# jperezrua/mfas

Measured on AMD Instinct MI355X. Metric: candidate-archs trained/sec (NTU inner loop), higher is better.
Workload: dtype f32

## Files before the change

mfas_amd/csrc/chain.hip.h:

```cpp
#pragma once
struct ChainArgs {
    const CandDev* cands;
    float* plane;
    int64_t plane_stride;
    const float* wt;
    float* stepbuf;
    mfas_table tab;
    const int32_t* order;
    int64_t pos_t;
    int32_t base_t, nvalid;
    int32_t gstep, epoch, E;
    int32_t yf_in_lds, vec_in_lds;
    AdamC ac;
    Geo g;
    DevStats* stats;
    int32_t* status;
    const float* pos_w;
    uint32_t* cellflag;
    uint32_t flag_target, _padf;
    int32_t yf_reduced, _padr;
    float* logits_out;
    const float* dlogits_in;
    float* xch;
    int32_t xpar, nsplit, ncand, _pads;
// ... 1514 lines not shown
template <int MB>
__device__ __forceinline__ void lean_res_load(const ChainArgs& a, const int bid, float* lds, LeanRes& rs) {
    const CandDev& cd = a.cands[bid];
    const LeanLds<MB> ll(lds, a.g);
    const int tid = threadIdx.x, lane = tid & 63, wave = tid >> 6;
    for (int e = tid; e < ll.nvec; e += CHAIN_THREADS)
        for (int pl = 0; pl < 3; ++pl) ll.vec_l[pl * ll.nvec + e] = a.plane[pl * a.plane_stride + cd.vec_off + e];
    if (wave < LEAN_OWN_TILES) {
        const int s = wave;
        const bool live = lean_own_live(cd, a.g, s);
        for (int pl = 0; pl < 3; ++pl) {
            f32x4 v = {0.f, 0.f, 0.f, 0.f};
            if (live) v = *reinterpret_cast<const f32x4*>(a.plane + pl * a.plane_stride + lean_own_off(cd, s) + lane * 4);
            *reinterpret_cast<f32x4*>(ll.own + (pl * LEAN_OWN_TILES + s) * 256 + lane * 4) = v;
        }
        f32x4 t = {0.f, 0.f, 0.f, 0.f};
        if (live) t = *reinterpret_cast<const f32x4*>(a.wt + lean_own_toff(cd, s) + lane * 4);
        *reinterpret_cast<f32x4*>(ll.own + (3 * LEAN_OWN_TILES + s) * 256 + lane * 4) = t;
    }
    if (tid == CHAIN_THREADS - 64) { rs.loss = 0.0; rs.corr = 0; rs.bad = 0; }
    if (tid < 16) reinterpret_cast<uint32_t*>(ll.scr + LEAN_BNF)[tid] = 0u;
    __syncthreads();
}

template <int MB>
__device__ __forceinline__ void lean_res_update(const ChainArgs& a, const ChainStep& cs, const int bid, float* lds) {
    const CandDev& cd = a.cands[bid];
    const Geo& g = a.g;
    const LeanLds<MB> ll(lds, g);
    constexpr int Bp = MB * 16, SX = 20;
    const int tid = threadIdx.x, lane = tid & 63, wave = tid >> 6;
    const int l15 = lane & 15, lg = lane >> 4;
    const int L = cd.L;
    int s = -1;
    const float* x = nullptr;
    const float* dy = nullptr;
    int sx = SX, sd = SX, dcol = 0;
    if (wave >= 1 && wave < L) { s = wave - 1; x = ll.xo_l + (wave - 1) * Bp * SX; dy = ll.dy_l + wave * Bp * SX; }
    else if (wave >= 4 && wave - 4 < g.ncb) { s = 3 + (wave - 4); x = ll.xo_l + (L - 1) * Bp * SX; dy = ll.lg_l; sd = ll.SC; dcol = (wave - 4) * 16; }
    if (s >= 0) {
        float* oW = ll.own + s * 256 + lane * 4;
        float* oM = oW + LEAN_OWN_TILES * 256;
        float* oV = oM + LEAN_OWN_TILES * 256;
        f32x4 w4 = *reinterpret_cast<const f32x4*>(oW), m4 = *reinterpret_cast<const f32x4*>(oM), v4 = *reinterpret_cast<const f32x4*>(oV);
        f32x4 acc = {0.f, 0.f, 0.f, 0.f};
        DW_BATCH_LOOP(MB, (g.B + 3) >> 2, acc = MFMA16(x[(4 * j + lg) * sx + l15], dy[(4 * j + lg) * sd + dcol + l15], acc))
        const float gsc = 1.0f;
        adam4(w4, m4, v4, acc * gsc, cs.ss, cs.bc2s, a.ac.w1, a.ac.b2, a.ac.w2, a.ac.eps, a.ac.wd);
        *reinterpret_cast<f32x4*>(oW) = w4;
        *reinterpret_cast<f32x4*>(oM) = m4;
        *reinterpret_cast<f32x4*>(oV) = v4;
        float* oT = ll.own + (3 * LEAN_OWN_TILES + s) * 256;
        const int base = (((l15 >> 2) * 16 + 4 * lg) << 2) + (l15 & 3);
#pragma unroll
        for (int q = 0; q < 4; ++q) oT[base + 4 * q] = w4[q];
    }
    lds_barrier();
}

template <int MB>
__device__ __forceinline__ void lean_res_store(const ChainArgs& a, const int bid, const int epoch, float* lds, const LeanRes& rs) {
    const CandDev& cd = a.cands[bid];
    const LeanLds<MB> ll(lds, a.g);
    const int tid = threadIdx.x, lane = tid & 63, wave = tid >> 6;
    __syncthreads();
    for (int e = tid; e < ll.nvec; e += CHAIN_THREADS)
        for (int pl = 0; pl < 3; ++pl) a.plane[pl * a.plane_stride + cd.vec_off + e] = ll.vec_l[pl * ll.nvec + e];
    if (wave < LEAN_OWN_TILES && lean_own_live(cd, a.g, wave)) {
        const int s = wave;
        for (int pl = 0; pl < 3; ++pl)
            *reinterpret_cast<f32x4*>(a.plane + pl * a.plane_stride + lean_own_off(cd, s) + lane * 4) =
                *reinterpret_cast<const f32x4*>(ll.own + (pl * LEAN_OWN_TILES + s) * 256 + lane * 4);
        *reinterpret_cast<f32x4*>(const_cast<float*>(a.wt) + lean_own_toff(cd, s) + lane * 4) =
            *reinterpret_cast<const f32x4*>(ll.own + (3 * LEAN_OWN_TILES + s) * 256 + lane * 4);
    }
    if (tid == CHAIN_THREADS - 64) {
        DevStats& st = a.stats[(int64_t)cd.gidx * a.E + epoch];
        st.train_loss += rs.loss;
        st.train_corr += rs.corr;
        if (rs.bad) atomicMax(&a.status[cd.gidx], 1);
    }
}

#define XCH_SLOTS 7
#define XCH_SENT 0xFFFFFFFFu
#define XCH_SPIN_LIMIT (1u << 21)
#define XCH_CAND_FLOATS (2 * XCH_SLOTS * 8 * 256)

__device__ __forceinline__ f32x4 xch_wait(const float* base, const int64_t idx, int32_t* status, const int gidx) {
    uint32_t spins = 0;
    for (;;) {
        const f32x4 v = ldc4<true>(base, idx);
        const u32x4 u = __builtin_bit_cast(u32x4, v);
        if (u[0] != XCH_SENT && u[1] != XCH_SENT && u[2] != XCH_SENT && u[3] != XCH_SENT) return v;
        if (++spins > XCH_SPIN_LIMIT) { atomicMax(&status[gidx], 2); return v; }
        asm volatile("" ::: "memory");
        __builtin_amdgcn_s_sleep(1);
    }
}

template <int NS> __host__ __device__ constexpr size_t chain_split_lds_floats(int Rp, int Cp) {
    return (size_t)2 * 16 * (Rp + 4) + (size_t)16 * (Cp + 4) + (size_t)MFAS_MAX_CELLS * (8 / NS) * 16 + 48 + 16 +
           (size_t)MFAS_MAX_CELLS * (8 / NS) * 256 + (size_t)(MFAS_MAX_CELLS * 5 * (8 / NS) * 16 + Cp) + (size_t)(8 / NS) * 8 * 256 +
           (size_t)2 * MFAS_MAX_CELLS * (8 / NS) * 256 + (size_t)(8 / NS) * 256;
}

template <int NS>
__device__ __forceinline__ void chain_split(const ChainArgs& a, const ChainStep& cs, const int bid, const int part, float* lds) {
#ifdef MFAS_CHAIN_TIMING
    const unsigned long long ct0 = __builtin_readcyclecounter();
#define CS_STAMP(slot) do { if (threadIdx.x == 0 && bid == 0 && part == 0 && cs.gstep == 3) a.status[64 + (slot)] = (int32_t)(__builtin_readcyclecounter() - ct0); } while (0)
    if (threadIdx.x == 0 && bid == 0 && part == 0 && (cs.gstep == 3 || cs.gstep == 4)) a.status[64 + 23 + 2 * (cs.gstep - 3)] = (int32_t)wall_clock64();
#else
#define CS_STAMP(slot) do { } while (0)
#endif
    constexpr int NRO = 8 / NS;
    constexpr int Bp = 16, MB = 1;
    const CandDev& cd = a.cands[bid];
    const Geo& g = a.g;
    const int tid = threadIdx.x, lane = tid & 63, wave = tid >> 6;
    const int l15 = lane & 15, lg = lane >> 4;
    const int Rp = g.Rp, nrb = 8, Cp = g.Cp, ncb = g.ncb, R = g.R, C = g.C, L = cd.L;
    const int SX = Rp + 4, SC = Cp + 4;
    constexpr int LPR = 16;
    float* xo_l = lds;
    float* dy_l = xo_l;
    float* lg_l = xo_l + 2 * Bp * SX;
    float* rstd_l = lg_l + Bp * SC;
    float* red_l = rstd_l + MFAS_MAX_CELLS * (8 / NS) * 16;
    int* lab_l = reinterpret_cast<int*>(red_l + 48);
    float* yf_l = reinterpret_cast<float*>(lab_l + 16);
    constexpr int NCOL = NRO * 16;
    float* vl = yf_l + MFAS_MAX_CELLS * NRO * 256;
    const int nvec = MFAS_MAX_CELLS * 5 * NCOL;
    const int vplane = nvec + Cp;
    float* tb = vl + vplane;
    float* sv_l = tb + NRO * 8 * 256;
    float* odd_l = sv_l + 2 * MFAS_MAX_CELLS * NRO * 256;

    float* W = a.plane;
    float* Mv = a.plane + a.plane_stride;
    float* Vv = Mv + a.plane_stride;
    float* sb = a.stepbuf + cd.step_off;
    const int64_t cvec_off = cd.vec_off;
    int nlbits = 0;
#pragma unroll
    for (int i = 0; i < MFAS_MAX_CELLS; ++i) nlbits |= (cd.conf[i][2] & 3) << (2 * i);
    const int cgidx = cd.gidx;
    asm volatile("" :: "s"(nlbits), "s"(cgidx));
    CS_STAMP(34);
    const int64_t oP1 = cd.seg_off[1][2], oP2 = cd.seg_off[2][2], oP3 = cd.seg_off[3][2];
    const int64_t oT1 = cd.outT_off[1], oT2 = cd.outT_off[2], oT3 = cd.outT_off[3], oHT = cd.headT_off;
    auto offP = [&](const int i) { return i == 1 ? oP1 : (i == 2 ? oP2 : oP3); };
    auto offT = [&](const int i) { return i == 1 ? oT1 : (i == 2 ? oT2 : oT3); };
    const int nvalid = cs.nvalid;
    const float nf = (float)nvalid;
    const AdamC ac = adam_consts(a.ac, cs.ss, cs.bc2s);
    const uint32_t h0 = lowbias32(cd.drop_seed + 0x9E3779B9U * (uint32_t)(cs.gstep + 1));
    const int64_t sbo = cd.step_off;
    const int rb0 = part * NRO;
    const bool main_w = wave < NRO;
    const int rb = rb0 + (main_w ? wave : 0);
    const int64_t xq = (int64_t)cgidx * XCH_CAND_FLOATS;
    const int64_t xcur_par = xq + (int64_t)a.xpar * (XCH_SLOTS * 8 * 256);
    const int64_t xoth_par = xq + (int64_t)(a.xpar ^ 1) * (XCH_SLOTS * 8 * 256);

    f32x4 hw[4];
    const int hcb = wave & 3, hpar = wave >> 2;
    const bool head_w = hcb < ncb;
#pragma unroll
    for (int u = 0; u < 4; ++u) {
        hw[u] = (f32x4){0.f, 0.f, 0.f, 0.f};
        if (head_w) hw[u] = *reinterpret_cast<const f32x4*>(W + cd.head_off + ((int64_t)hcb * nrb + 2 * u + hpar) * 256 + lane * 4);
    }
    f32x4 stg[NRO];
    auto stage_issue = [&](const float* base, const int64_t off0, const int nk) {
#pragma unroll
        for (int u = 0; u < NRO; ++u) {
            const int e = wave + 8 * u;
            const int j = e / nk, k = e - j * nk;
            if (e < NRO * nk) stg[u] = *reinterpret_cast<const f32x4*>(base + off0 + ((int64_t)(rb0 + j) * nk + k) * 256 + lane * 4);
        }
    };
    auto stage_store = [&](float* dst, const int nk) {
#pragma unroll
        for (int u = 0; u < NRO; ++u) {
            const int e = wave + 8 * u;
            const int j = e / nk, k = e - j * nk;
            if (e < NRO * nk) *as_lds(reinterpret_cast<f32x4*>(dst + (j * 8 + k) * 256 + lane * 4)) = stg[u];
        }
// ... 86 lines not shown
            const int u = 2 * u2 + odd;
            if (u < nk) {
                const f32x4 w4 = *as_lds(reinterpret_cast<const f32x4*>(tiles + u * 256 + lane * 4));
                const f32x4 x4 = *reinterpret_cast<const f32x4*>(X + l15 * sx + u * 16 + 4 * lg);
#pragma unroll
                for (int q = 0; q < 4; ++q) acc = MFMA16(x4[q], w4[q], acc);
            }
        }
    };
    const bool help_w = wave >= NRO && wave < 2 * NRO;
    static_assert(2 * (8 / NS) <= 4, "main + helper waves below the head waves");
    const int vcol = (main_w ? wave : 0) * 16 + l15;

    for (int i = 0; i < L; ++i) {
        CS_STAMP(1 + i);
        if (i == L - 1 && lab_b >= 0 && lab_b < Bp && lab_b < nvalid) lab_r = g.loss_mode == 0 ? a.tab.label[lab_row] : (int)lab_row;
        const bool st_fw = i + 1 < L && i >= 1;
        const bool st_hd = i + 1 == L;
        if (st_fw) stage_issue(W, offP(i + 1), nrb);
        else if (st_hd) stage_issue(a.wt, oHT, ncb);
        const float* xprev = xo_l + ((i + 1) & 1) * Bp * SX;
        float* xcur = xo_l + (i & 1) * Bp * SX;
        if (main_w) {
            const int nl = (nlbits >> (2 * i)) & 3;
            const int64_t vb = cvec_off + (int64_t)i * g.vec_cell_stride;
            const float* vc = vl + i * 5 * NCOL;
            const int r = rb * 16 + l15;
            const bool colok = r < R;
            const float bias = vc[VEC_B * NCOL + vcol];
            float gam = 1.f, bet = 0.f;
            if (g.bn) { gam = vc[VEC_G * NCOL + vcol]; bet = vc[VEC_BE * NCOL + vcol]; }
            f32x4 acc = *as_lds(reinterpret_cast<const f32x4*>(yf_l + ((i * NRO + wave) << 8) + lane * 4));
            if (i > 0) {
                mma_half(acc, xprev, SX, tb + wave * 8 * 256, nrb, 0);
                lds_barrier();
                acc += *as_lds(reinterpret_cast<const f32x4*>(odd_l + wave * 256 + lane * 4));
            }
            if (i == 1) CS_STAMP(13);
            float av[4];
            float s = 0.f;
#pragma unroll
            for (int q = 0; q < 4; ++q) {
                const int b = 4 * lg + q;
                const float v = act_fwd(acc[q] + bias, nl);
                av[q] = v;
                if (b < nvalid) s += v;
            }
            float zv[4];
            if (g.bn) {
                const float mu = colsum(s) / nf;
                float s2 = 0.f;
#pragma unroll
                for (int q = 0; q < 4; ++q) {
                    const int b = 4 * lg + q;
                    const float dlt = av[q] - mu;
                    if (b < nvalid) s2 += dlt * dlt;
                }
                const float var = colsum(s2) / nf;
                const float rstd = 1.0f / sqrtf(var + g.bn_eps);
                f32x4 xh4;
#pragma unroll
                for (int q = 0; q < 4; ++q) {
                    const float xh = (av[q] - mu) * rstd;
                    xh4[q] = xh;
                    zv[q] = xh * gam + bet;
                }
                if (lg == 0) {
                    rstd_l[i * NCOL + vcol] = rstd;
                    if (colok) {
                        float rm = vc[VEC_RM * NCOL + vcol], rv = vc[VEC_RV * NCOL + vcol];
                        const float unb = var * (nf / (nf - 1.0f));
                        rm += g.bn_mom * (mu - rm);
                        rv += g.bn_mom * (unb - rv);
                        W[vb + VEC_RM * Rp + r] = rm;
                        W[vb + VEC_RV * Rp + r] = rv;
                    }
                }
                *as_lds(reinterpret_cast<f32x4*>(sv_l + ((MFAS_MAX_CELLS + i) * NRO + wave) * 256 + lane * 4)) = xh4;
            } else {
#pragma unroll
                for (int q = 0; q < 4; ++q) zv[q] = av[q];
            }
            *as_lds(reinterpret_cast<f32x4*>(sv_l + (i * NRO + wave) * 256 + lane * 4)) = (f32x4){av[0], av[1], av[2], av[3]};
            float* xo_g = sb + g.sb_xo + (int64_t)i * Bp * Rp;
            f32x4 o4;
#pragma unroll
            for (int q = 0; q < 4; ++q) {
                const int b = 4 * lg + q;
                float o = zv[q];
                if (g.use_drop) o = ((keepm >> (4 * i + q)) & 1u) ? o * g.drop_scale : 0.0f;
                if (!(colok && b < nvalid)) o = 0.0f;
                o4[q] = o;
            }
            stc4<true>(a.xch, xcur_par + ((int64_t)i * 8 + rb) * 256 + lane * 4, o4);
            if (i == 1) CS_STAMP(14);
            if (i + 1 < L) keep_bits(i + 1);
#pragma unroll
            for (int q = 0; q < 4; ++q) {
                const int b = 4 * lg + q;
                xcur[b * SX + r] = o4[q];
                stc1<true>(xo_g + b * Rp + r, o4[q]);
            }
        }
        if (!main_w && i > 0) {
            if (help_w) {
                f32x4 acc2 = {0.f, 0.f, 0.f, 0.f};
                mma_half(acc2, xprev, SX, tb + (wave - NRO) * 8 * 256, nrb, 1);
                *as_lds(reinterpret_cast<f32x4*>(odd_l + (wave - NRO) * 256 + lane * 4)) = acc2;
            }
            lds_barrier();
        }
        if (st_fw) stage_store(tb, nrb);
        else if (st_hd) stage_store(tb, ncb);
        if (i == 1) CS_STAMP(15);
        fetch_others(i, xcur);
        if (i == 1) CS_STAMP(16);
        lds_barrier();
    }

    CS_STAMP(5);
    {
        const float* xl = xo_l + ((L - 1) & 1) * Bp * SX;
        float* hodd = xo_l + (L & 1) * Bp * SX;
        f32x4 acc = {0.f, 0.f, 0.f, 0.f};
        if (head_w) {
#pragma unroll
            for (int u = 0; u < 4; ++u) {
                const f32x4 x4 = *reinterpret_cast<const f32x4*>(xl + l15 * SX + (2 * u + hpar) * 16 + 4 * lg);
#pragma unroll
                for (int q = 0; q < 4; ++q) acc = MFMA16(x4[q], hw[u][q], acc);
            }
            if (hpar) *as_lds(reinterpret_cast<f32x4*>(hodd + hcb * 256 + lane * 4)) = acc;
        }
        lds_barrier();
        if (head_w && !hpar) {
            acc += *as_lds(reinterpret_cast<const f32x4*>(hodd + hcb * 256 + lane * 4));
            const int c = hcb * 16 + l15;
            const float bias = vl[nvec + c];
#pragma unroll
            for (int q = 0; q < 4; ++q) lg_l[(4 * lg + q) * SC + c] = acc[q] + bias;
        }
    }
    if (lab_b >= 0 && lab_b < Bp) lab_l[lab_b] = lab_r;
    lds_barrier();
    CS_STAMP(6);
    if (g.loss_mode == 1) {
        if (tid < 4 * Bp) bce_rows(lg_l, SC, red_l, Bp, lab_l, a.tab.multilabel, a.pos_w, C, Cp, nvalid, tid);
    } else if (Cp <= 64 && !g.multitask) {
        if (tid < 8 * Bp) softmax_rows_lean<MB>(a, lg_l, SC, red_l, lab_l, nvalid, nf, tid);
    } else if (tid < LPR * Bp) {
        softmax_rows<MB>(a, cs, lg_l, SC, red_l, lab_l, nvalid, nf, tid, cand_order(a.order, g, cgidx));
    }
    CS_STAMP(21);
    lds_barrier();
    if (part == 0) {
        if (tid == CHAIN_THREADS - 64 && a.stats) {
            float ls = 0.f, ncor = 0.f;
            for (int b = 0; b < Bp; ++b) { ls += red_l[b]; ncor += red_l[Bp + b]; }
            DevStats& st = a.stats[(int64_t)cgidx * a.E + cs.epoch];
            st.train_loss += (double)ls;
            st.train_corr += (long long)ncor;
            if (!(fabsf(ls) <= 3.0e38f)) atomicMax(&a.status[cgidx], 1);
        }
        float* dlg = sb + g.sb_dlog;
        for (int e = tid; e < Bp * Cp; e += CHAIN_THREADS) {
            const int b = e / Cp, c = e - b * Cp;
            stc1<true>(dlg + e, lg_l[b * SC + c]);
        }
        const int hc = tid - (CHAIN_THREADS - 256);
        if (hc >= 0 && hc < C) {
            float gsum = 0.f;
            for (int b = 0; b < Bp; ++b) gsum += lg_l[b * SC + hc];
            const int64_t o = cvec_off + g.vec_head + hc;
            float w = vl[nvec + hc], m = Mv[o], v = Vv[o];
            adam1(w, m, v, gsum, ac);
            W[o] = w; Mv[o] = m; Vv[o] = v;
        }
    }
    CS_STAMP(7);

    for (int i = L - 1; i >= 0; --i) {
        CS_STAMP(8 + (L - 1 - i));
        const int j = L - 1 - i;
        const bool st_bw = i >= 1;
        if (st_bw) stage_issue(a.wt, offT(i), nrb);
        const bool from_head = (i == L - 1);
        const float* src = from_head ? lg_l : dy_l + ((i + 1) & 1) * Bp * SX;
        const int sstride = from_head ? SC : SX;
        const int nkk = from_head ? ncb : nrb;
        float* dcur = dy_l + (i & 1) * Bp * SX;
        if (main_w) {
            const int nl = (nlbits >> (2 * i)) & 3;
            const int64_t vb = cvec_off + (int64_t)i * g.vec_cell_stride;
            const float* vc = vl + i * 5 * NCOL;
            const int r = rb * 16 + l15;
            const bool colok = r < R;
            float gr = 0.f;
            if (g.bn) gr = vc[VEC_G * NCOL + vcol] * rstd_l[i * NCOL + vcol];
            const int64_t ob = vb + VEC_B * Rp + r, og = vb + VEC_G * Rp + r, obe = vb + VEC_BE * Rp + r;
            float pw[3] = {0.f, 0.f, 0.f}, pm[3] = {0.f, 0.f, 0.f}, pv[3] = {0.f, 0.f, 0.f};
            if (lg == 0 && colok) {
                pw[0] = vc[VEC_B * NCOL + vcol]; pm[0] = Mv[ob]; pv[0] = Vv[ob];
                if (g.bn) {
                    pw[1] = vc[VEC_G * NCOL + vcol]; pm[1] = Mv[og]; pv[1] = Vv[og];
                    pw[2] = vc[VEC_BE * NCOL + vcol]; pm[2] = Mv[obe]; pv[2] = Vv[obe];
                }
            }
            const f32x4 a4 = *as_lds(reinterpret_cast<const f32x4*>(sv_l + (i * NRO + wave) * 256 + lane * 4));
            f32x4 xh4 = {0.f, 0.f, 0.f, 0.f};
            if (g.bn) xh4 = *as_lds(reinterpret_cast<const f32x4*>(sv_l + ((MFAS_MAX_CELLS + i) * NRO + wave) * 256 + lane * 4));
            f32x4 acc = {0.f, 0.f, 0.f, 0.f};
            mma_half(acc, src, sstride, tb + wave * 8 * 256, nkk, 0);
            lds_barrier();
            acc += *as_lds(reinterpret_cast<const f32x4*>(odd_l + wave * 256 + lane * 4));
            if (i == 2) CS_STAMP(17);
            float dz[4];
            float sdz = 0.f, sdzx = 0.f;
#pragma unroll
            for (int q = 0; q < 4; ++q) {
                const int b = 4 * lg + q;
                float d = acc[q];
                if (g.use_drop) d = ((keepm >> (4 * i + q)) & 1u) ? d * g.drop_scale : 0.0f;
                if (!(b < nvalid)) d = 0.f;
                dz[q] = d;
                sdz += d;
                if (g.bn) sdzx += d * xh4[q];
            }
            float dgam = 0.f, dbet = 0.f;
            if (g.bn) {
                dbet = colsum(sdz);
                dgam = colsum(sdzx);
                const float k1 = dbet / nf, k2 = dgam / nf;
#pragma unroll
                for (int q = 0; q < 4; ++q) {
                    const int b = 4 * lg + q;
                    const float da = gr * (dz[q] - k1 - xh4[q] * k2);
                    dz[q] = b < nvalid ? da : 0.f;
                }
            }
            float sdy = 0.f;
            float* dy_g = sb + g.sb_dy + (int64_t)i * Bp * Rp;
            f32x4 d4;
#pragma unroll
            for (int q = 0; q < 4; ++q) {
                float dy = act_bwd(a4[q], dz[q], nl);
                if (!colok) dy = 0.f;
                sdy += dy;
                d4[q] = dy;
            }
            if (i >= 1) stc4<true>(a.xch, xcur_par + ((int64_t)(4 + j) * 8 + rb) * 256 + lane * 4, d4);
            if (i == 2) CS_STAMP(18);
#pragma unroll
            for (int q = 0; q < 4; ++q) {
                const int b = 4 * lg + q;
                dcur[b * SX + r] = d4[q];
                stc1<true>(dy_g + b * Rp + r, d4[q]);
            }
            const float db = colsum(sdy);
            if (lg == 0 && colok) {
                adam1(pw[0], pm[0], pv[0], db, ac);
                W[ob] = pw[0]; Mv[ob] = pm[0]; Vv[ob] = pv[0];
                if (g.bn) {
                    adam1(pw[1], pm[1], pv[1], dgam, ac);
                    W[og] = pw[1]; Mv[og] = pm[1]; Vv[og] = pv[1];
                    adam1(pw[2], pm[2], pv[2], dbet, ac);
                    W[obe] = pw[2]; Mv[obe] = pm[2]; Vv[obe] = pv[2];
                }
            }
        }
        if (!main_w) {
            if (help_w) {
                f32x4 acc2 = {0.f, 0.f, 0.f, 0.f};
                mma_half(acc2, src, sstride, tb + (wave - NRO) * 8 * 256, nkk, 1);
                *as_lds(reinterpret_cast<f32x4*>(odd_l + (wave - NRO) * 256 + lane * 4)) = acc2;
            }
            lds_barrier();
        }
        if (st_bw) stage_store(tb, nrb);
        if (i == 2) CS_STAMP(19);
        if (i >= 1) fetch_others(4 + j, dcur);
        if (i == 2) CS_STAMP(20);
        asm volatile("s_waitcnt vmcnt(0)" ::: "memory");
        lds_barrier();
        if (a.cellflag && tid == 0)
            __hip_atomic_fetch_add(a.cellflag + (size_t)cgidx * CELLFLAG_STRIDE + i, 1u, __ATOMIC_RELAXED, __HIP_MEMORY_SCOPE_AGENT);
    }
    CS_STAMP(12);
#ifdef MFAS_CHAIN_TIMING
    if (threadIdx.x == 0 && bid == 0 && part == 0 && (cs.gstep == 3 || cs.gstep == 4)) a.status[64 + 24 + 2 * (cs.gstep - 3)] = (int32_t)wall_clock64();
#endif
#undef CS_STAMP
}
```

mfas_amd/csrc/common.hip.h:

```cpp
#pragma once

typedef float f32x4 __attribute__((ext_vector_type(4)));
typedef int32_t i32x4 __attribute__((ext_vector_type(4)));
typedef uint32_t u32x4 __attribute__((ext_vector_type(4)));
typedef uint32_t u32x2 __attribute__((ext_vector_type(2)));
#define MFAS_LDS __attribute__((address_space(3)))
#define MFAS_GLB __attribute__((address_space(1)))
template <typename T> __device__ __forceinline__ MFAS_LDS T* as_lds(T* p) { return (MFAS_LDS T*)p; }
template <typename T> __device__ __forceinline__ MFAS_GLB T* as_glb(T* p) { return (MFAS_GLB T*)p; }
#define MFMA16(a, b, c) __builtin_amdgcn_mfma_f32_16x16x4f32((a), (b), (c), 0, 0, 0)

#define KIND_S 0
#define KIND_V 1
#define KIND_OUT 2
#define KIND_HEAD 3

static thread_local std::string g_err;
static int fail(int code, const std::string& msg) {
    g_err = msg;
    return code;
}
#define HIPCHK(x)                                                                                  \
    do {                                                                                           \
        hipError_t e_ = (x);                                                                       \
// ... 247 lines not shown
    if (dtype == MFAS_DT_F32) {
        const int vpr = ncols >> 2;
        for (int e = tid; e < nrows * vpr; e += nthreads) {
            const int b = e / vpr, c = (e - b * vpr) << 2;
            f32x4 val = {0.f, 0.f, 0.f, 0.f};
            if (b < nvalid) {
                const int64_t row = ord ? (int64_t)ord[pos + b] : (int64_t)(base + b);
                val = *reinterpret_cast<const f32x4*>(reinterpret_cast<const float*>(tab) + row * width + col0 + c);
            }
            *as_lds(reinterpret_cast<f32x4*>(dst + b * stride + c)) = val;
        }
    } else {
        const int vpr = ncols >> 3;
        for (int e = tid; e < nrows * vpr; e += nthreads) {
            const int b = e / vpr, c = (e - b * vpr) << 3;
            f32x4 lo = {0.f, 0.f, 0.f, 0.f}, hi = {0.f, 0.f, 0.f, 0.f};
            if (b < nvalid) {
                const int64_t row = ord ? (int64_t)ord[pos + b] : (int64_t)(base + b);
                const uint4 raw = *reinterpret_cast<const uint4*>(reinterpret_cast<const uint16_t*>(tab) +
                                                                  row * width + col0 + c);
                const uint32_t w[4] = {raw.x, raw.y, raw.z, raw.w};
                float f[8];
#pragma unroll
                for (int j = 0; j < 4; ++j) {
                    if (dtype == MFAS_DT_BF16) {
                        f[2 * j] = __uint_as_float(w[j] << 16);
                        f[2 * j + 1] = __uint_as_float(w[j] & 0xFFFF0000U);
                    } else {
                        f[2 * j] = __half2float(__ushort_as_half((unsigned short)(w[j] & 0xFFFFU)));
                        f[2 * j + 1] = __half2float(__ushort_as_half((unsigned short)(w[j] >> 16)));
                    }
                }
                lo = (f32x4){f[0], f[1], f[2], f[3]};
                hi = (f32x4){f[4], f[5], f[6], f[7]};
            }
            *as_lds(reinterpret_cast<f32x4*>(dst + b * stride + c)) = lo;
            *as_lds(reinterpret_cast<f32x4*>(dst + b * stride + c + 4)) = hi;
        }
    }
}

typedef unsigned u32x4 __attribute__((ext_vector_type(4)));
#define MFAS_AUX_SC1 16
__device__ __forceinline__ __amdgpu_buffer_rsrc_t mk_rsrc(const float* base) {
    return __builtin_amdgcn_make_buffer_rsrc(const_cast<float*>(base), 0, -1, 0x00020000);
}
template <bool COH>
__device__ __forceinline__ f32x4 ldc4(const float* base, int64_t idx) {
    if constexpr (COH) {
        const u32x4 r = __builtin_amdgcn_raw_buffer_load_b128(mk_rsrc(base), (int)(uint32_t)(idx << 2), 0, MFAS_AUX_SC1);
        return __builtin_bit_cast(f32x4, r);
    } else {
        return *reinterpret_cast<const f32x4*>(base + idx);
    }
}
template <bool COH>
__device__ __forceinline__ void stc4(float* base, int64_t idx, f32x4 v) {
    if constexpr (COH)
        __builtin_amdgcn_raw_buffer_store_b128(__builtin_bit_cast(u32x4, v), mk_rsrc(base), (int)(uint32_t)(idx << 2), 0, MFAS_AUX_SC1);
    else
        *reinterpret_cast<f32x4*>(base + idx) = v;
}
template <bool COH>
__device__ __forceinline__ void stc1(float* p, float v) {
    if constexpr (COH) __hip_atomic_store(p, v, __ATOMIC_RELAXED, __HIP_MEMORY_SCOPE_AGENT);
    else *p = v;
}
template <bool COH>
__device__ __forceinline__ float ldc1(const float* p) {
    if constexpr (COH) return __hip_atomic_load(p, __ATOMIC_RELAXED, __HIP_MEMORY_SCOPE_AGENT);
    else return *p;
}

template <bool COH>
__device__ __forceinline__ void stage_f32(float* dst, int stride, const float* base, int64_t idx0, int src_stride, int ncols,
                                          int nrows, int tid, int nthreads) {
    const int vpr = ncols >> 2;
    for (int e = tid; e < nrows * vpr; e += nthreads) {
        const int b = e / vpr, c = (e - b * vpr) << 2;
        *reinterpret_cast<f32x4*>(dst + b * stride + c) = ldc4<COH>(base, idx0 + (int64_t)b * src_stride + c);
    }
}

template <int MB, int WPE> struct SweepU { static constexpr int v = (MB == 2 && WPE == 4) ? 1 : 2; };
```

mfas_amd/csrc/mfas_hip.hip:

```cpp
#include <hip/hip_runtime.h>
#include <hip/hip_fp16.h>
#pragma clang fp contract(off)
#include <stdint.h>
#include <stdio.h>
#include <string.h>
#include <math.h>
#include <algorithm>
#include <string>
#include <vector>
#include <thread>
#include <chrono>
#include <dlfcn.h>

#include "mfas_hip.h"

#include "common.hip.h"
#include "sweep.hip.h"
#include "chain.hip.h"

struct StepArgs {
    SweepArgs sa;
    ChainArgs ca;
    int32_t nchain, _pad;
    GatherArgs ga;
};

template <int MB, bool NT, int WPE, bool LEAN, int NS = 1>
__global__ void __launch_bounds__(STEP_THREADS, WPE) k_step(const StepArgs a) {
    extern __shared__ __attribute__((aligned(16))) float lds[];
    const int bid = (int)blockIdx.x;
    if (bid < a.nchain) {
        if constexpr (NS > 1) {
            const int Kp = a.nchain / NS, part = bid / Kp, c = bid - part * Kp;
            if (c < a.ca.ncand) chain_split<NS>(a.ca, chain_step_of(a.ca), c, part, lds);
        } else
        if constexpr (LEAN) { chain_lean<MB, 0, (WPE >= 4 ? 8 : 16)>(a.ca, chain_step_of(a.ca), bid, lds, lean_pre<MB>(a.ca, bid)); chain_lean_tail<MB, 0>(a.ca, chain_step_of(a.ca), bid, lds); }
        else chain_body<MB, false>(a.ca, chain_step_of(a.ca), bid, lds);
    }
    else if (bid < a.nchain + a.ga.nblocks) gather_body(a.ga, a.ga.cands[bid - a.nchain], a.sa.g, a.sa.tab, a.sa.order, (int)threadIdx.x);
    else if (bid < a.nchain + a.ga.nblocks + a.sa.ntap) sweep_tap_body<MB, NT, SweepU<MB, WPE>::v>(a.sa, bid - a.nchain - a.ga.nblocks, lds);
    else sweep_body<MB, NT, SweepU<MB, WPE>::v>(a.sa, sweep_step_of(a.sa), bid - a.nchain - a.ga.nblocks - a.sa.ntap, lds);
}

template <int MB, bool NT, int NS = 1>
__global__ void __launch_bounds__(STEP_THREADS, 4) k_step_same(const StepArgs a) {
    extern __shared__ __attribute__((aligned(16))) float lds[];
    const int bid = (int)blockIdx.x;
    if (bid < a.nchain) {
        if constexpr (NS > 1) {
            const int Kp = a.nchain / NS, part = bid / Kp, c = bid - part * Kp;
            if (c < a.ca.ncand) chain_split<NS>(a.ca, chain_step_of(a.ca), c, part, lds);
        } else chain_body<MB, false, true>(a.ca, chain_step_of(a.ca), bid, lds);
    } else sweep_body<MB, NT, SweepU<MB, 4>::v, true>(a.sa, sweep_step_of(a.sa), bid - a.nchain, lds);
}

template <int MB, bool LEAN>
__global__ void __launch_bounds__(STEP_THREADS, 2) k_chain(const ChainArgs a) {
    extern __shared__ __attribute__((aligned(16))) float lds[];
    if constexpr (LEAN) { chain_lean<MB>(a, chain_step_of(a), (int)blockIdx.x, lds, lean_pre<MB>(a, (int)blockIdx.x)); chain_lean_tail<MB, 0>(a, chain_step_of(a), (int)blockIdx.x, lds); }
    else chain_body<MB, true>(a, chain_step_of(a), (int)blockIdx.x, lds);
}

#include "wide.hip.h"
#include "persist.hip.h"
#include "eval.hip.h"
#include "pack.hip.h"

#include "plan.hip.h"

struct mfas_population {
    mfas_hyper hp;
    Tuning tune;
    int K = 0, device = 0, n_cus = 0;
    int chunk_cols_req = 0;
    hipStream_t stream = nullptr;
    LayoutPlan plan;
    float* plane = nullptr;
    float* wt = nullptr;
    float* stepbuf = nullptr;
    float* best = nullptr;
    CandDev* d_cands = nullptr;
    SegDesc* d_descs = nullptr;
    struct GroupDev { SegDesc* d_descs = nullptr; TapDesc* d_taps = nullptr; };
    std::vector<GroupDev> groups;
    DevStats* d_stats = nullptr;
    int32_t* d_status = nullptr;
    uint32_t* d_seeds = nullptr;
    long long* d_corr = nullptr;
    float* d_posw = nullptr;
    int stats_cap = 0;
    bool profiling = false;
    int prof_every = 16;
    std::vector<hipEvent_t> ev;
    int64_t prof_launches = 0;
    double prof_ms = 0.0, bytes_per_launch = 0.0, prof_bytes = 0.0;
    double best_threshold = 0.0;
    struct Progress {
        std::vector<int64_t> done, nb;
        std::vector<double> best_metric;
        std::vector<int32_t> keeps_best;
        void reset(int K, double threshold) { done.assign(K, 0); nb.assign(K, 0); best_metric.assign(K, threshold); keeps_best.assign(K, 0); }
    } prog;
    float* d_move = nullptr;
    int64_t move_cap = 0;
    uint32_t* d_red_cnt = nullptr;
    char* d_gather = nullptr;
    size_t gather_cap = 0;
    uint32_t* d_cellflag = nullptr;
    float* d_xch = nullptr;
    SegDesc* d_pdescs = nullptr;
    int fell_back = 0;
    uint32_t* d_sync = nullptr;
    int32_t* d_need = nullptr;
    int32_t* d_role = nullptr;
    float* d_scal = nullptr;
    size_t scal_cap = 0;
    unsigned long long* d_trace = nullptr;
};

namespace {
struct Roctx {
    int (*push)(const char*) = nullptr;
    int (*pop)() = nullptr;
    Roctx() {
        if (getenv("MFAS_NO_ROCTX")) return;
        void* h = dlopen("librocprofiler-sdk-roctx.so", RTLD_LAZY | RTLD_LOCAL);
        if (!h) h = dlopen("librocprofiler-sdk-roctx.so.1", RTLD_LAZY | RTLD_LOCAL);
        if (!h) h = dlopen("libroctx64.so", RTLD_LAZY | RTLD_LOCAL);
        if (!h) return;
        push = reinterpret_cast<int (*)(const char*)>(dlsym(h, "roctxRangePushA"));
        pop = reinterpret_cast<int (*)()>(dlsym(h, "roctxRangePop"));
        if (!push || !pop) { push = nullptr; pop = nullptr; }
    }
};
Roctx& roctx() { static Roctx r; return r; }
struct RangeGuard {
// ... 460 lines not shown
```

mfas_amd/csrc/sweep.hip.h:

```cpp
#pragma once
template <int MB, bool NT, int SWEEP_U, bool COH = false>
__device__ __forceinline__ void tile_run(float* Wp, float* Mp, float* Vp, const int rb, const int nkb, const int kb0,
                                         const int kbs, const float* xt, const int ST, const float* xn, const int SN,
                                         const float (&dyf)[MB * 4], const float gsc, const AdamC& ac, const bool upd,
                                         const bool fwd, f32x4 (&yacc)[MB], float* T, const int tstride_rb,
                                         const int lane, const int nj) {
    const int l15 = lane & 15, lg = lane >> 4;
    const float a_ss = ac.ss, a_bc2s = ac.bc2s, a_w1 = ac.w1, a_b2 = ac.b2, a_w2 = ac.w2, a_eps = ac.eps, a_wd = ac.wd;
    for (int kbb = kb0; kbb < nkb; kbb += SWEEP_U * kbs) {
        f32x4 w4[SWEEP_U], m4[SWEEP_U], v4[SWEEP_U];
#pragma unroll
        for (int u = 0; u < SWEEP_U; ++u) {
            const int kb = kbb + u * kbs;
            if (kb < nkb) {
                const int64_t off = ((int64_t)rb * nkb + kb) * 256 + lane * 4;
                w4[u] = NT ? __builtin_nontemporal_load(reinterpret_cast<const f32x4*>(Wp + off))
                           : *reinterpret_cast<const f32x4*>(Wp + off);
                if (upd) {
                    m4[u] = NT ? __builtin_nontemporal_load(reinterpret_cast<const f32x4*>(Mp + off))
                               : *reinterpret_cast<const f32x4*>(Mp + off);
                    v4[u] = NT ? __builtin_nontemporal_load(reinterpret_cast<const f32x4*>(Vp + off))
                               : *reinterpret_cast<const f32x4*>(Vp + off);
                }
            }
// ... 69 lines not shown
__device__ __forceinline__ int64_t gather_tap_off(const Geo& g, const int kind, const int tap, const int eb) {
    int64_t o = 0;
#pragma unroll
    for (int u = 0; u < MFAS_MAX_TAPS; ++u) {
        if (kind == KIND_V || u < tap) o += g.sw[u];
        if (kind == KIND_V && u < tap) o += g.vw[u];
    }
    return o * g.Bp * eb;
}

struct GatherArgs {
    const CandDev* cands;
    char* buf;
    int64_t cand_stride, par_stride;
    int64_t pos[2];
    int32_t base[2], nvalid[2], par[2];
    int32_t nsets, nblocks;
};

__device__ __forceinline__ void gather_body(const GatherArgs& ga, const CandDev& cd, const Geo& g, const mfas_table& tab,
                                            const int32_t* order, const int tid) {
    const int eb = tab.dtype == MFAS_DT_F32 ? 4 : 2;
    const int32_t* ordp = cand_order(order, g, cd.gidx);
    uint32_t used = 0;
    for (int i = 0; i < cd.L; ++i) used |= (1u << cd.conf[i][0]) | (1u << (MFAS_MAX_TAPS + cd.conf[i][1]));
#pragma unroll
    for (int s = 0; s < 2; ++s) {
        if (s >= ga.nsets) break;
        char* dst0 = ga.buf + (int64_t)cd.gidx * ga.cand_stride + (int64_t)ga.par[s] * ga.par_stride;
        for (int kt = 0; kt < 2 * MFAS_MAX_TAPS; ++kt) {
            if (!((used >> kt) & 1u)) continue;
            const int kind = kt < MFAS_MAX_TAPS ? KIND_S : KIND_V, tap = kt & (MFAS_MAX_TAPS - 1);
            const int w = kind == KIND_S ? g.sw[tap] : g.vw[tap];
            const char* src0 = reinterpret_cast<const char*>(kind == KIND_S ? tab.s[tap] : tab.v[tap]);
            char* dst = dst0 + gather_tap_off(g, kind, tap, eb);
            const int vpr = (w * eb) >> 4, nvec = ga.nvalid[s] * vpr;
            for (int e0 = tid; e0 < nvec; e0 += 4 * STEP_THREADS) {
                u32x4 v[4];
#pragma unroll
                for (int u = 0; u < 4; ++u) {
                    const int e = e0 + u * STEP_THREADS;
                    if (e < nvec) {
                        const int b = e / vpr, c = e - b * vpr;
                        const int64_t row = ordp ? (int64_t)ordp[ga.pos[s] + b] : (int64_t)(ga.base[s] + b);
                        v[u] = *reinterpret_cast<const u32x4*>(src0 + (row * w) * eb + ((int64_t)c << 4));
                    }
                }
#pragma unroll
                for (int u = 0; u < 4; ++u) {
                    const int e = e0 + u * STEP_THREADS;
                    if (e < nvec) {
                        const int b = e / vpr, c = e - b * vpr;
                        *reinterpret_cast<u32x4*>(dst + ((int64_t)b * w) * eb + ((int64_t)c << 4)) = v[u];
                    }
                }
            }
        }
    }
}

struct SweepStep {
    int64_t pos_t, pos_n;
    int32_t base_t, base_n, nvalid_t, nvalid_n;
    int32_t upd, fwd;
    float ss, bc2s;
};
__device__ __forceinline__ SweepStep sweep_step_of(const SweepArgs& a) {
    SweepStep s;
    s.pos_t = a.pos_t; s.pos_n = a.pos_n; s.base_t = a.base_t; s.base_n = a.base_n;
    s.nvalid_t = a.nvalid_t; s.nvalid_n = a.nvalid_n; s.upd = a.do_update; s.fwd = a.do_forward;
    s.ss = a.ac.ss; s.bc2s = a.ac.bc2s;
    return s;
}


#ifdef MFAS_CHAIN_TIMING
#define SW_UNIT_STAMP(k) do { if (COH && a.cellflag && a.flag_target == 16u && threadIdx.x == 0 && d.cell == 0 && d.kind == KIND_S && d.k0 == 0 && d.cand == 0) a.flag_status[64 + 29 + (k)] = (int32_t)wall_clock64(); } while (0)
#define SW_END_STAMP() do { if (COH && a.cellflag && a.flag_target == 16u && threadIdx.x == 0) { atomicMax(reinterpret_cast<uint32_t*>(&a.flag_status[64 + 27]), (uint32_t)wall_clock64()); \
        atomicMax(reinterpret_cast<uint32_t*>(&a.flag_status[128 + d.cell * 4 + d.kind]), (uint32_t)wall_clock64()); } } while (0)
#else
#define SW_END_STAMP() do { } while (0)
#define SW_UNIT_STAMP(k) do { } while (0)
#endif
template <int MB, bool NT, int U, bool COH = false>
__device__ __forceinline__ void sweep_body(const SweepArgs& a, const SweepStep& st, const int bid, float* lds) {
    const SegDesc d = a.desc[bid];
    const CandDev& cd = a.cands[d.cand];
    const int tid = threadIdx.x, lane = tid & 63, wave = tid >> 6;
    const int l15 = lane & 15, lg = lane >> 4;
    constexpr int Bp = MB * 16;
    const int cc = d.cc, rows_p = d.rows_p, nrb = rows_p >> 4, nkb = cc >> 4;
    const int ST = cc + 16;
    const int SN = cc + 4;
    const int SD = rows_p + 16;
    float* xt = lds;
    float* xn = xt + Bp * ST;
    float* dyl = xn + Bp * SN;
    float* wred = dyl + Bp * SD;
    const bool feat = d.kind <= KIND_V;
    const bool upd = st.upd != 0;
    const bool fwd = (st.fwd != 0) && feat;
    if (!upd && !fwd) return;
    const int64_t sbo = cd.step_off;
    const bool red = a.red_cnt != nullptr;

    if (!COH && a.gather && feat) {
        const char* gb = a.gather + (int64_t)cd.gidx * a.g_cand_stride + gather_tap_off(a.g, d.kind, d.tap, a.tab.dtype == MFAS_DT_F32 ? 4 : 2);
        if (upd) stage_table(xt, ST, gb + (int64_t)a.g_par_t * a.g_par_stride, a.tab.dtype, d.width, d.k0, cc, nullptr, 0, 0, st.nvalid_t, Bp, tid, STEP_THREADS);
        if (fwd) stage_table(xn, SN, gb + (int64_t)a.g_par_n * a.g_par_stride, a.tab.dtype, d.width, d.k0, cc, nullptr, 0, 0, st.nvalid_n, Bp, tid, STEP_THREADS);
    } else {
    if (upd && feat) {
        const void* tp = d.kind == KIND_S ? a.tab.s[d.tap] : a.tab.v[d.tap];
        stage_table(xt, ST, tp, a.tab.dtype, d.width, d.k0, cc, cand_order(a.order, a.g, cd.gidx), st.pos_t, st.base_t, st.nvalid_t, Bp, tid, STEP_THREADS);
    }
    if (fwd) {
        const void* tp = d.kind == KIND_S ? a.tab.s[d.tap] : a.tab.v[d.tap];
        stage_table(xn, SN, tp, a.tab.dtype, d.width, d.k0, cc, cand_order(a.order, a.g, cd.gidx), st.pos_n, st.base_n, st.nvalid_n, Bp, tid, STEP_THREADS);
    }
    }
    if constexpr (COH) {
        if (upd && a.cellflag) {
            __shared__ int s_go;
            if (tid == 0) {
                const int slot = d.kind == KIND_HEAD ? cd.L - 1 : (d.kind == KIND_OUT ? d.cell - 1 : d.cell);
                const uint32_t* f = a.cellflag + (size_t)cd.gidx * CELLFLAG_STRIDE + slot;
                uint32_t spins = 0;
                int go = 1;
                while (ld_u32_relaxed(f) < a.flag_target) {
                    __builtin_amdgcn_s_sleep(2);
                    if (++spins > CELLFLAG_SPIN_LIMIT) { go = 0; atomicMax(&a.flag_status[cd.gidx], 2); break; }
                }
                s_go = go;
#ifdef MFAS_CHAIN_TIMING
                if (a.flag_target == 16u && slot == 0 && d.kind <= KIND_V) atomicMin(reinterpret_cast<uint32_t*>(&a.flag_status[64 + 28]), (uint32_t)wall_clock64());
#endif
            }
            __syncthreads();
            if (!s_go) return;
            SW_UNIT_STAMP(0);
        }
    }
    if (upd) {
        if (!feat) {
            const int xcell = d.kind == KIND_OUT ? d.cell - 1 : cd.L - 1;
            stage_f32<COH>(xt, ST, a.stepbuf, sbo + a.g.sb_xo + (int64_t)xcell * Bp * a.g.Rp + d.k0, a.g.Rp, cc, Bp, tid, STEP_THREADS);
        }
        const int64_t dsrc = d.kind == KIND_HEAD ? sbo + a.g.sb_dlog : sbo + a.g.sb_dy + (int64_t)d.cell * Bp * a.g.Rp;
        stage_f32<COH>(dyl, SD, a.stepbuf, dsrc + d.rb0 * 16, d.seg_nrb * 16, rows_p, Bp, tid, STEP_THREADS);
    }
    __syncthreads();
    SW_UNIT_STAMP(1);

    float* Wp = a.plane + d.w_off;
    float* Mp = Wp + a.plane_stride;
    float* Vp = Mp + a.plane_stride;
    const AdamC ac = adam_consts(a.ac, upd ? st.ss : 0.f, upd ? st.bc2s : 1.f);
    float gsc = 1.0f;
    if (a.g.alphas && feat && upd) gsc = ldc1<COH>(a.stepbuf + sbo + a.g.sb_gsc + d.cell * 2 + d.kind);

    const bool split_k = nrb < STEP_NW;
    const int rb0 = split_k ? 0 : wave, rbs = split_k ? 1 : STEP_NW;
    const int kb0 = split_k ? wave : 0, kbs = split_k ? STEP_NW : 1;
    const int64_t part = sbo + a.g.sb_part + (((int64_t)(cd.part_cell_off[d.cell] + d.part_idx) * d.seg_nrb * MB) << 8) +
                         (((int64_t)d.rb0 * MB) << 8);

    for (int rb = rb0; rb < nrb; rb += rbs) {
        float dyf[MB * 4];
#pragma unroll
        for (int j = 0; j < MB * 4; ++j) dyf[j] = upd ? dyl[(4 * j + lg) * SD + rb * 16 + l15] : 0.f;
        f32x4 yacc[MB];
#pragma unroll
        for (int mb = 0; mb < MB; ++mb) yacc[mb] = (f32x4){0.f, 0.f, 0.f, 0.f};
        tile_run<MB, NT, U, COH>(Wp, Mp, Vp, rb, nkb, kb0, kbs, xt, ST, xn, SN, dyf, gsc, ac, upd, fwd, yacc,
                                 d.wt_off >= 0 ? a.wt + d.wt_off + ((int64_t)(d.k0 >> 4) * d.seg_nrb + d.rb0) * 256 : nullptr, d.seg_nrb, lane, (a.g.B + 3) >> 2);
        if (fwd) {
#pragma unroll
            for (int mb = 0; mb < MB; ++mb) {
                if (split_k)
                    *reinterpret_cast<f32x4*>(wred + (((wave * nrb + rb) * MB + mb) << 8) + lane * 4) = yacc[mb];
                else if (red) stc4<true>(a.stepbuf, part + ((rb * MB + mb) << 8) + lane * 4, yacc[mb]);
                else
                    stc4<COH>(a.stepbuf, part + ((rb * MB + mb) << 8) + lane * 4, yacc[mb]);
            }
        }
    }
    SW_UNIT_STAMP(2);
    if (!fwd) { SW_END_STAMP(); return; }
    if (split_k) {
        __syncthreads();
        for (int e = tid; e < nrb * MB * 64; e += STEP_THREADS) {
            const int slot = e >> 6, ln = e & 63;
            f32x4 s = *reinterpret_cast<const f32x4*>(wred + (slot << 8) + ln * 4);
#pragma unroll
            for (int w = 1; w < STEP_NW; ++w)
                s += *reinterpret_cast<const f32x4*>(wred + ((w * nrb * MB + slot) << 8) + ln * 4);
            if (red) stc4<true>(a.stepbuf, part + (slot << 8) + ln * 4, s);
            else stc4<COH>(a.stepbuf, part + (slot << 8) + ln * 4, s);
        }
    }
    if (!red) { SW_END_STAMP(); return; }
    asm volatile("s_waitcnt vmcnt(0)" ::: "memory");
    __syncthreads();
    SW_UNIT_STAMP(3);
    int* flagw = reinterpret_cast<int*>(lds);
    const int ns_c = cd.nch_s[d.cell], nch_c = ns_c + cd.nch_v[d.cell];
    if (tid == 0) {
        uint32_t* cnt = a.red_cnt + d.cand * MFAS_MAX_CELLS + d.cell;
        const uint32_t old = __hip_atomic_fetch_add(cnt, 1u, __ATOMIC_RELAXED, __HIP_MEMORY_SCOPE_AGENT);
        const int last = old == (uint32_t)(nch_c - 1);
        if (last) __hip_atomic_store(cnt, 0u, __ATOMIC_RELAXED, __HIP_MEMORY_SCOPE_AGENT);
        flagw[0] = last;
    }
    __syncthreads();
    SW_UNIT_STAMP(4);
    if (!flagw[0]) { SW_END_STAMP(); return; }
    {
        const int snrb = d.seg_nrb;
        const int per_cell = snrb * MB * 64;
        const int64_t part0 = sbo + a.g.sb_part + (((int64_t)cd.part_cell_off[d.cell] * snrb * MB) << 8);
        const int64_t yf0 = sbo + a.g.sb_yf + (int64_t)d.cell * per_cell * 4;
        const int64_t vplane = (int64_t)MFAS_MAX_CELLS * snrb * MB * 256;
        for (int it = tid; it < per_cell; it += STEP_THREADS) {
            f32x4 accS = {0.f, 0.f, 0.f, 0.f}, accV = {0.f, 0.f, 0.f, 0.f};
            constexpr int PB = 8;
            for (int ch0 = 0; ch0 < nch_c; ch0 += PB) {
                f32x4 p8[PB];
#pragma unroll
                for (int u = 0; u < PB; ++u)
                    if (ch0 + u < nch_c) p8[u] = ldc4<true>(a.stepbuf, part0 + (((int64_t)(ch0 + u) * snrb * MB) << 8) + it * 4);
#pragma unroll
                for (int u = 0; u < PB; ++u)
// ... 63 lines not shown
```

Baseline: 35.14.

## Feed sweep from xch exchange buffer and drop redundant row stores in split chain

In the split-chain path, the per-row scalar stores of forward outputs and backward dy into the step buffer are removed. The sweep blocks instead stage those activations and gradients directly from the xch exchange buffer, which the chain already writes in 256-float tiles. XCH_SLOTS grows from 7 to 8 so that the cell-0 dy tile is also published, and a new tile-unpacking stage helper is added. This cuts duplicate global stores in the chain. The cost is a more complex cross-kernel data contract, with a risk of reading stale or mis-indexed slots.

```diff
diff --git a/mfas_amd/csrc/chain.hip.h b/mfas_amd/csrc/chain.hip.h
--- a/mfas_amd/csrc/chain.hip.h
+++ b/mfas_amd/csrc/chain.hip.h
@@ -1620,10 +1620,8 @@
     }
 }
 
-#define XCH_SLOTS 7
 #define XCH_SENT 0xFFFFFFFFu
 #define XCH_SPIN_LIMIT (1u << 21)
-#define XCH_CAND_FLOATS (2 * XCH_SLOTS * 8 * 256)
 
 __device__ __forceinline__ f32x4 xch_wait(const float* base, const int64_t idx, int32_t* status, const int gidx) {
     uint32_t spins = 0;
@@ -1643,7 +1641,7 @@
            (size_t)2 * MFAS_MAX_CELLS * (8 / NS) * 256 + (size_t)(8 / NS) * 256;
 }
 
-template <int NS>
+template <int NS, bool ROWS = true>
 __device__ __forceinline__ void chain_split(const ChainArgs& a, const ChainStep& cs, const int bid, const int part, float* lds) {
 #ifdef MFAS_CHAIN_TIMING
     const unsigned long long ct0 = __builtin_readcyclecounter();
@@ -1896,7 +1894,7 @@
                 for (int q = 0; q < 4; ++q) zv[q] = av[q];
             }
             *as_lds(reinterpret_cast<f32x4*>(sv_l + (i * NRO + wave) * 256 + lane * 4)) = (f32x4){av[0], av[1], av[2], av[3]};
-            float* xo_g = sb + g.sb_xo + (int64_t)i * Bp * Rp;
+            [[maybe_unused]] float* xo_g = sb + g.sb_xo + (int64_t)i * Bp * Rp;
             f32x4 o4;
 #pragma unroll
             for (int q = 0; q < 4; ++q) {
@@ -1913,7 +1911,7 @@
             for (int q = 0; q < 4; ++q) {
                 const int b = 4 * lg + q;
                 xcur[b * SX + r] = o4[q];
-                stc1<true>(xo_g + b * Rp + r, o4[q]);
+                if constexpr (ROWS) stc1<true>(xo_g + b * Rp + r, o4[q]);
             }
         }
         if (!main_w && i > 0) {
@@ -2053,7 +2051,7 @@
                 }
             }
             float sdy = 0.f;
-            float* dy_g = sb + g.sb_dy + (int64_t)i * Bp * Rp;
+            [[maybe_unused]] float* dy_g = sb + g.sb_dy + (int64_t)i * Bp * Rp;
             f32x4 d4;
 #pragma unroll
             for (int q = 0; q < 4; ++q) {
@@ -2062,13 +2060,13 @@
                 sdy += dy;
                 d4[q] = dy;
             }
-            if (i >= 1) stc4<true>(a.xch, xcur_par + ((int64_t)(4 + j) * 8 + rb) * 256 + lane * 4, d4);
+            if (i >= 1 || !ROWS) stc4<true>(a.xch, xcur_par + ((int64_t)(4 + j) * 8 + rb) * 256 + lane * 4, d4);
             if (i == 2) CS_STAMP(18);
 #pragma unroll
             for (int q = 0; q < 4; ++q) {
                 const int b = 4 * lg + q;
                 dcur[b * SX + r] = d4[q];
-                stc1<true>(dy_g + b * Rp + r, d4[q]);
+                if constexpr (ROWS) stc1<true>(dy_g + b * Rp + r, d4[q]);
             }
             const float db = colsum(sdy);
             if (lg == 0 && colok) {
diff --git a/mfas_amd/csrc/common.hip.h b/mfas_amd/csrc/common.hip.h
--- a/mfas_amd/csrc/common.hip.h
+++ b/mfas_amd/csrc/common.hip.h
@@ -353,4 +353,15 @@
     }
 }
 
+#define XCH_SLOTS 8
+#define XCH_CAND_FLOATS (2 * XCH_SLOTS * 8 * 256)
+__device__ __forceinline__ void stage_pieces(float* dst, int stride, const float* base, int64_t idx0, int nrbs, int tid, int nthreads) {
+    for (int e = tid; e < nrbs * 64; e += nthreads) {
+        const int prb = e >> 6, ln = e & 63;
+        const f32x4 v = ldc4<true>(base, idx0 + (int64_t)prb * 256 + ln * 4);
+#pragma unroll
+        for (int q = 0; q < 4; ++q) dst[(4 * (ln >> 4) + q) * stride + prb * 16 + (ln & 15)] = v[q];
+    }
+}
+
 template <int MB, int WPE> struct SweepU { static constexpr int v = (MB == 2 && WPE == 4) ? 1 : 2; };
diff --git a/mfas_amd/csrc/mfas_hip.hip b/mfas_amd/csrc/mfas_hip.hip
--- a/mfas_amd/csrc/mfas_hip.hip
+++ b/mfas_amd/csrc/mfas_hip.hip
@@ -49,9 +49,10 @@
     if (bid < a.nchain) {
         if constexpr (NS > 1) {
             const int Kp = a.nchain / NS, part = bid / Kp, c = bid - part * Kp;
-            if (c < a.ca.ncand) chain_split<NS>(a.ca, chain_step_of(a.ca), c, part, lds);
+            if (c < a.ca.ncand) chain_split<NS, false>(a.ca, chain_step_of(a.ca), c, part, lds);
         } else chain_body<MB, false, true>(a.ca, chain_step_of(a.ca), bid, lds);
-    } else sweep_body<MB, NT, SweepU<MB, 4>::v, true>(a.sa, sweep_step_of(a.sa), bid - a.nchain, lds);
+    } else sweep_body<MB, NT, SweepU<MB, 4>::v, true, (NS > 1)>(a.sa, sweep_step_of(a.sa), bid - a.nchain, lds, a.ca.xch,
+                                                                (int64_t)a.ca.xpar * (XCH_SLOTS * 8 * 256));
 }
 
 template <int MB, bool LEAN>
diff --git a/mfas_amd/csrc/sweep.hip.h b/mfas_amd/csrc/sweep.hip.h
--- a/mfas_amd/csrc/sweep.hip.h
+++ b/mfas_amd/csrc/sweep.hip.h
@@ -175,8 +175,9 @@
 #define SW_END_STAMP() do { } while (0)
 #define SW_UNIT_STAMP(k) do { } while (0)
 #endif
-template <int MB, bool NT, int U, bool COH = false>
-__device__ __forceinline__ void sweep_body(const SweepArgs& a, const SweepStep& st, const int bid, float* lds) {
+template <int MB, bool NT, int U, bool COH = false, bool XD = false>
+__device__ __forceinline__ void sweep_body(const SweepArgs& a, const SweepStep& st, const int bid, float* lds,
+                                           const float* xch = nullptr, const int64_t xpar_off = 0) {
     const SegDesc d = a.desc[bid];
     const CandDev& cd = a.cands[d.cand];
     const int tid = threadIdx.x, lane = tid & 63, wave = tid >> 6;
@@ -234,12 +235,15 @@
         }
     }
     if (upd) {
+        const int64_t xq = xpar_off + (int64_t)cd.gidx * XCH_CAND_FLOATS;
         if (!feat) {
             const int xcell = d.kind == KIND_OUT ? d.cell - 1 : cd.L - 1;
-            stage_f32<COH>(xt, ST, a.stepbuf, sbo + a.g.sb_xo + (int64_t)xcell * Bp * a.g.Rp + d.k0, a.g.Rp, cc, Bp, tid, STEP_THREADS);
+            if constexpr (XD) stage_pieces(xt, ST, xch, xq + ((int64_t)xcell * 8 + (d.k0 >> 4)) * 256, nkb, tid, STEP_THREADS);
+            else stage_f32<COH>(xt, ST, a.stepbuf, sbo + a.g.sb_xo + (int64_t)xcell * Bp * a.g.Rp + d.k0, a.g.Rp, cc, Bp, tid, STEP_THREADS);
         }
         const int64_t dsrc = d.kind == KIND_HEAD ? sbo + a.g.sb_dlog : sbo + a.g.sb_dy + (int64_t)d.cell * Bp * a.g.Rp;
-        stage_f32<COH>(dyl, SD, a.stepbuf, dsrc + d.rb0 * 16, d.seg_nrb * 16, rows_p, Bp, tid, STEP_THREADS);
+        if (XD && d.kind != KIND_HEAD) stage_pieces(dyl, SD, xch, xq + ((int64_t)(4 + cd.L - 1 - d.cell) * 8 + d.rb0) * 256, nrb, tid, STEP_THREADS);
+        else stage_f32<COH>(dyl, SD, a.stepbuf, dsrc + d.rb0 * 16, d.seg_nrb * 16, rows_p, Bp, tid, STEP_THREADS);
     }
     __syncthreads();
     SW_UNIT_STAMP(1);
```

Measured after the change: 35.09. About the same (-0.1%).
